# SuwoongHeo/neurecon

Hardware: AMD Instinct MI355X
Metric: rays/sec (4096 rays x 128 samples, 8-layer x256 SDF MLP) (higher is better)
Workload: dtype f16x3

## Files before the change

### neurecon_amd/csrc/nr_mlp.hip

```cpp
#include <algorithm>
#include <atomic>
#include <type_traits>
#include "nr_common.h"
#include "nr_mlp.h"
#include "nr_tgemm.h"

namespace nr {

using lds_ptr = __attribute__((address_space(3))) void*;

__device__ __forceinline__ void glds16(const char* gsrc, uint32_t lds_addr) {
  unsigned keep;
  asm volatile(
      "s_mov_b32 %0, m0\n\t"
      "s_mov_b32 m0, %2\n\t"
      "s_nop 0\n\t"
      "global_load_lds_dwordx4 %1, off\n\t"
      "s_mov_b32 m0, %0"
      : "=&s"(keep)
      : "v"(gsrc), "s"(lds_addr)
      : "memory");
}

__device__ __forceinline__ void glds16s(const char* sbase, uint32_t voff, uint32_t lds_addr) {
// ... 725 lines not shown
template <bool DERIV>
__device__ __forceinline__ void softplus3(float z, float& y, float& s) {
  const float t = z * 100.0f;
  const bool lin = t > 20.0f;
  const float ex = __builtin_amdgcn_exp2f(t * 1.44269504088896341f);
  const float u = 1.0f + ex;
  const float yy = __builtin_amdgcn_logf(u) * (0.693147180559945309f * 0.01f);
  y = lin ? z : yy;
  if constexpr (DERIV) s = lin ? 1.0f : ex * __builtin_amdgcn_rcpf(u);
}
__device__ __forceinline__ void softplus1(float z, float& y, float& s) {
  const float t = z * 144.269504088896341f;
  const float ex = __builtin_amdgcn_exp2f(t);
  const float u = ex + 1.0f;
  const bool lin = t > 28.8539008f;
  y = lin ? z : __builtin_amdgcn_logf(u) * (0.693147180559945309f * 0.01f);
  s = lin ? 1.0f : ex * __builtin_amdgcn_rcpf(u);
}
template <bool DERIV>
__device__ __forceinline__ void softplus_pk(float z0, float z1, float& y0, float& y1, float& s0, float& s1) {
  float d0, d1;
  softplus1(z0, y0, d0);
  softplus1(z1, y1, d1);
  if constexpr (DERIV) {
    s0 = d0;
    s1 = d1;
  }
}
__device__ __forceinline__ float4 fma4s(f32x4 a, float m, float4 b) {
  return make_float4(__builtin_fmaf(a[0], m, b.x), __builtin_fmaf(a[1], m, b.y), __builtin_fmaf(a[2], m, b.z),
                     __builtin_fmaf(a[3], m, b.w));
}

using gf4 = __attribute__((address_space(1))) f32x4;

constexpr int kNC = 1;
constexpr int kW4 = 8 / kNC;
constexpr int kT4 = 64 * kW4;
constexpr int kWPE = kW4 / 4;
constexpr int kSlabW = 2 * kNC * 1024;
constexpr int kSlab4 = kW4 * kSlabW;
constexpr int kLoad = 8;
static_assert(kLoad >= 1 && kLoad <= kW4, "loader waves");

typedef uint32_t u32x3 __attribute__((ext_vector_type(3)));
struct Pend4 {
  float4* base;
  uint32_t o[4];
  float4 v[4];
  int n;
  bool nt;
  bool b96;
  __device__ __forceinline__ int flush() {
    int issued = 0;
    if (base) {
      issued = n;
#pragma unroll
      for (int i = 0; i < 4; ++i) {
        if (i < n) {
          if (b96) {
            const uint32_t off = o[i];
            const u32x3 d = {__float_as_uint(v[i].x), __float_as_uint(v[i].y), __float_as_uint(v[i].z)};
            if (nt) asm volatile("global_store_dwordx3 %0, %1, %2 nt\n\ts_nop 1" : : "v"(off), "v"(d), "s"(base) : "memory");
            else asm volatile("global_store_dwordx3 %0, %1, %2\n\ts_nop 1" : : "v"(off), "v"(d), "s"(base) : "memory");
          } else {
            const uint32_t off = o[i] * 16u;
            const f32x4 d = tof(v[i]);
            if (nt) asm volatile("global_store_dwordx4 %0, %1, %2 nt\n\ts_nop 1" : : "v"(off), "v"(d), "s"(base) : "memory");
            else asm volatile("global_store_dwordx4 %0, %1, %2\n\ts_nop 1" : : "v"(off), "v"(d), "s"(base) : "memory");
          }
        }
      }
      base = nullptr;
    }
    return issued;
  }
  __device__ __forceinline__ void put(float4* b, int cnt, bool nontemporal, bool bytes96 = false) {
    base = b;
    n = cnt;
    nt = nontemporal;
    b96 = bytes96;
  }
};

constexpr int kSlabRing = 3;
constexpr int kFwdRing = 4;
constexpr int kTabBytes = 8 * 512;
constexpr bool kSlabNT = true;
constexpr bool kFeatNT = false;

template <int CBMAX, int RING = 3, int NW = kW4>
struct WStream4 {
  static_assert(RING == 3 || RING == 4, "weight ring depth");
  static constexpr int kRingN = RING;
  static constexpr int kLd = NW == kW4 ? kLoad : NW;
  char* lds;
  char* slab;
  int cur;
  int es;
  int er;
  int prev;
  char* tab;
  int tcur;
  __device__ __forceinline__ static int wave_id() { return __builtin_amdgcn_readfirstlane(threadIdx.x >> 6); }
  __device__ __forceinline__ static int next3(int i) { return i == 2 ? 0 : i + 1; }
  __device__ __forceinline__ static int nextr(int i) { return i == RING - 1 ? 0 : i + 1; }
  __device__ __forceinline__ int ahead_slot() const { return cur == 0 ? RING - 1 : cur - 1; }
  template <int BYTES>
  __device__ __forceinline__ static constexpr int pieces() { return (BYTES / 1024 + kLd - 1) / kLd; }
  __device__ __forceinline__ static int loader() { return wave_id() - (NW - kLd); }
  template <int BYTES>
  __device__ __forceinline__ static int npieces() { return loader() >= 0 ? pieces<BYTES>() : 0; }
  template <int BYTES>
  __device__ __forceinline__ void dma(const char* gsrc, int slot) {
    constexpr int NB = BYTES / 1024, NPW = pieces<BYTES>();
    const int wave = loader();
    if (wave < 0) return;
    const uint32_t voff = (threadIdx.x & 63) * 16;
    const int first = __builtin_amdgcn_readfirstlane(min(wave * NPW, NB - NPW));
    const char* g = uniform_ptr(gsrc) + first * 1024;
    const uint32_t base =
        __builtin_amdgcn_readfirstlane(lds_u32(lds) + (uint32_t)(slot * CBMAX) + (uint32_t)(first * 1024));
#pragma unroll
    for (int j = 0; j < NPW; j += 4) {
      const char* gj = g + j * 1024;
      const uint32_t mj = base + j * 1024;
      if (NPW - j >= 4)
        asm volatile(
            "s_mov_b32 m0, %2\n\ts_nop 0\n\t"
            "global_load_lds_dwordx4 %0, %1\n\t"
            "global_load_lds_dwordx4 %0, %1 offset:1024\n\t"
            "global_load_lds_dwordx4 %0, %1 offset:2048\n\t"
            "global_load_lds_dwordx4 %0, %1 offset:3072"
            :
            : "v"(voff), "s"(gj), "s"(mj)
            : "memory", "m0");
      else if (NPW - j == 3)
        asm volatile(
            "s_mov_b32 m0, %2\n\ts_nop 0\n\t"
            "global_load_lds_dwordx4 %0, %1\n\t"
            "global_load_lds_dwordx4 %0, %1 offset:1024\n\t"
            "global_load_lds_dwordx4 %0, %1 offset:2048"
            :
            : "v"(voff), "s"(gj), "s"(mj)
            : "memory", "m0");
      else if (NPW - j == 2)
        asm volatile(
            "s_mov_b32 m0, %2\n\ts_nop 0\n\t"
            "global_load_lds_dwordx4 %0, %1\n\t"
            "global_load_lds_dwordx4 %0, %1 offset:1024"
            :
            : "v"(voff), "s"(gj), "s"(mj)
            : "memory", "m0");
      else
        glds16m(gj, voff, mj);
    }
  }
  template <int B0, int B1>
  __device__ __forceinline__ void start(const char* g0, const char* g1) {
    static_assert(RING == 3, "start: the first RING - 1 chunks");
    cur = 0;
    es = 0;
    er = 0;
    prev = 0;
    dma<B0>(g0, 0);
    dma<B1>(g1, 1);
// ... 69 lines not shown
    return (const float4*)(lds + off);
  }
  __device__ __forceinline__ void flip(int n) {
    if constexpr (RING == 4) {
      wait_vmcnt(n + prev);
      prev = n;
    } else {
      wait_vmcnt(n);
    }
    __syncthreads();
    cur = nextr(cur);
  }
  __device__ __forceinline__ void flip_nowait() {
    __syncthreads();
    cur = nextr(cur);
  }
};

__device__ __forceinline__ f16x8 rd_frag(const float4* __restrict__ A, int i, int lane) {
  return as_h8(A[i * 64 + lane]);
}
template <int NS, class Stage>
__device__ __forceinline__ void mma4(const float4* __restrict__ A, const f16x8 (&bh)[kNC][12],
                                     const f16x8 (&bl)[kNC][12], f32x4 (&acc)[kNC][2], int lane, Stage&& stage) {
  f16x8 nh0 = rd_frag(A, 0, lane), nl0 = rd_frag(A, 1, lane);
  f16x8 nh1 = rd_frag(A, NS * 2, lane), nl1 = rd_frag(A, NS * 2 + 1, lane);
#pragma unroll
  for (int s = 0; s < NS; ++s) {
    const f16x8 h0 = nh0, l0 = nl0, h1 = nh1, l1 = nl1;
    if (s + 1 < NS) {
      nh0 = rd_frag(A, (s + 1) * 2, lane);
      nl0 = rd_frag(A, (s + 1) * 2 + 1, lane);
      nh1 = rd_frag(A, (NS + s + 1) * 2, lane);
      nl1 = rd_frag(A, (NS + s + 1) * 2 + 1, lane);
    }
    stage(s);
#pragma unroll
    for (int q = 0; q < kNC; ++q) {
      acc[q][0] = mfma16h(l0, bh[q][s], acc[q][0]);
      acc[q][1] = mfma16h(l1, bh[q][s], acc[q][1]);
      acc[q][0] = mfma16h(h0, bl[q][s], acc[q][0]);
      acc[q][1] = mfma16h(h1, bl[q][s], acc[q][1]);
      acc[q][0] = mfma16h(h0, bh[q][s], acc[q][0]);
      acc[q][1] = mfma16h(h1, bh[q][s], acc[q][1]);
    }
    if (s + 1 < NS) __builtin_amdgcn_sched_group_barrier(0x100, 4, 0);
    __builtin_amdgcn_sched_group_barrier(0x008, 6 * kNC, 0);
    __builtin_amdgcn_sched_barrier(0);
  }
}

struct Z4 {
  float4 z[kNC][2];
  float4 aux[2];
};

constexpr float kT = 144.26944f;
constexpr float kC = 0.0069314749f;

#ifdef NR_EXP_STAMPS
constexpr int kStampPh = 9;
constexpr int kStampSlot = 2048 * 8 * kStampPh;
__device__ unsigned long long g_nr_stamps[6 * kStampSlot];
__device__ __forceinline__ unsigned long long* stamp_lds() {
  __shared__ unsigned long long s_stamp[kW4 * kStampPh];
  return s_stamp;
}
__device__ __forceinline__ uint64_t stamp_now() { return __builtin_amdgcn_s_memtime(); }
__device__ __forceinline__ void stamp_add(int ph, uint64_t dt) {
  if ((threadIdx.x & 63) == 0) stamp_lds()[(threadIdx.x >> 6) * kStampPh + ph] += dt;
}
#define NR_STAMP(var) const uint64_t var = stamp_now()
#define NR_STAMP_VAR(var) uint64_t var = 0
#define NR_STAMP_SET(var) var = stamp_now()
#define NR_STAMP_ADD(ph, dt) stamp_add(ph, dt)
#else
#define NR_STAMP(var)
#define NR_STAMP_VAR(var)
#define NR_STAMP_SET(var)
#define NR_STAMP_ADD(ph, dt)
#endif

enum { kSlot = 0, kLean = 1, kTab = 2 };
template <int KB, int NBO, int NXT_CB, bool AUX, bool TS, int MODE = kSlot, int NXT_MODE = kSlot, class WS,
          class Pre, class Epi>
__device__ __forceinline__ void op4(WS& ws, const char* __restrict__ op, const char* nxt, const f16x8 (&bh)[kNC][12],
                                    const f16x8 (&bl)[kNC][12], const float (&xinv)[kNC], Pend4& pd, Pre&& pre,
                                    Epi&& epi, int lane, float winv = 0.0f) {
  constexpr int CB = chunk_bytes(KB);
  constexpr bool LEAN = MODE == kLean;
  constexpr int FB = MODE != kSlot ? weight_bytes(KB) : CB;
  constexpr int NXT_FB = NXT_MODE != kSlot ? NXT_CB - 1024 : NXT_CB;
  static_assert(!LEAN || (!AUX && !TS), "lean ops carry no per-row data");
  constexpr int NCH = NBO / 2;
  static_assert(MODE != kTab || NCH * 512 <= kTabBytes, "bias table entries");
  constexpr int LA = WS::kRingN - 1;
  static_assert(NCH >= 2, "the 2-ahead stream needs >= 2 chunks per op");
  const int g = lane >> 4;
  Z4 zq{};
#pragma unroll
  for (int c = 0; c < NCH; ++c) {
    const char* opc = op;
    const char* nxc = nxt;
    asm volatile("" : "+s"(opc), "+s"(nxc));
    NR_STAMP(t0);
    int npend = 0;
    if (c + LA < NCH) {
      ws.template issue<FB>(opc + (c + LA) * CB);
      npend = WS::template npieces<FB>();
    } else if (nxc) {
      ws.template issue<NXT_FB>(nxc + (c + LA - NCH) * NXT_CB);
      npend = WS::template npieces<NXT_FB>();
      if constexpr (NXT_MODE == kTab) {
        if (c + LA == NCH) {
          ws.template dma_tab<NXT_CB>(nxc, ws.tcur ^ 1);
          npend += WS::ntab();
        }
      }
    }
    npend += pre(c);
    npend += pd.flush();
    NR_STAMP(t1);
    const float4* A = ws.buf();
    f32x4 acc[kNC][2] = {};
    mma4<KB / 2>(A, bh, bl, acc, lane, [&](int st) {
      if (c > 0) {
#pragma unroll
        for (int e = 0; e < 8; ++e)
          if (e * (KB / 2) / 8 == st) epi(c - 1, zq, e);
      }
    });
    NR_STAMP(t2);
    float wi;
    float4 b0, b1;
    if constexpr (LEAN) {
      wi = winv;
      b0 = b1 = make_float4(0.f, 0.f, 0.f, 0.f);
    } else {
      const float4* S = MODE == kTab ? ws.tab_entry(c) : A + 2 * KB * 64;
      wi = S[8].x;
      if constexpr (TS) wi *= kT;
      b0 = S[(TS ? 24 : 0) + g];
      b1 = S[(TS ? 28 : 4) + g];
    }
#pragma unroll
    for (int q = 0; q < kNC; ++q) {
      const float inv = xinv[q] * wi;
      zq.z[q][0] = fma4s(acc[q][0], inv, b0);
      zq.z[q][1] = fma4s(acc[q][1], inv, b1);
    }
    if constexpr (AUX) {
      const float4* S = MODE == kTab ? ws.tab_entry(c) : A + 2 * KB * 64;
      zq.aux[0] = S[16 + g];
      zq.aux[1] = S[20 + g];
    }
#ifdef NR_EXP_STAMPS
    wait_vmcnt(npend);
    NR_STAMP(t3);
    ws.flip(npend);
    NR_STAMP(t4);
    stamp_add(0, t1 - t0);
    stamp_add(1, t2 - t1);
    stamp_add(2, t3 - t2);
    stamp_add(3, t4 - t3);
    stamp_add(4, 1);
#else
    ws.flip(npend);
#endif
  }
  pd.flush();
  if constexpr (MODE == kTab) ws.tcur ^= 1;
#pragma unroll
  for (int e = 0; e < 8; ++e) epi(NCH - 1, zq, e);
}

template <bool NABLA>
__device__ __forceinline__ void sp_pair(const Z4& zz, int q, int k, float4 (&y)[2], float4& s0, float4& s1) {
  const int o = k >> 1;
  const float4 z = zz.z[q][o];
  float4& s = o ? s1 : s0;
  if ((k & 1) == 0) softplus_pk<NABLA>(z.x, z.y, y[o].x, y[o].y, s.x, s.y);
  else softplus_pk<NABLA>(z.z, z.w, y[o].z, y[o].w, s.z, s.w);
}
__device__ __forceinline__ float4 mul4(float4 a, float4 b) { return make_float4(a.x * b.x, a.y * b.y, a.z * b.z, a.w * b.w); }
__device__ __forceinline__ uint32_t opaque_lane(int lane) {
  uint32_t l = (uint32_t)lane;
  asm volatile("" : "+v"(l));
  return l;
}
__device__ __forceinline__ void pend_chunk(Pend4& pd, float4* base, int first_blk, int lane, bool nt) {
  const uint32_t l = opaque_lane(lane);
#pragma unroll
  for (int i = 0; i < 2 * kNC; ++i) pd.o[i] = (kNC * first_blk + i) * 64 + l;
  pd.put(base, 2 * kNC, nt);
}
__device__ __forceinline__ void pend_chunk24(Pend4& pd, float4* layer, int c, int lane, bool nt) {
  const uint32_t l = opaque_lane(lane);
#pragma unroll
  for (int i = 0; i < 2 * kNC; ++i) pd.o[i] = (uint32_t)(c * kNC * kSlab24Chunk) + ((uint32_t)i * 64 + l) * 12u;
  pd.put(layer, 2 * kNC, nt, true);
}
__device__ __forceinline__ uint32_t code24(float c) { return (uint32_t)__builtin_fmaf(c, 8388608.0f, 0.5f); }
__device__ __forceinline__ float4 pack24(float c0, float c1, float c2, float c3) {
  const uint32_t u0 = code24(c0), u1 = code24(c1), u2 = code24(c2), u3 = code24(c3);
  return make_float4(__uint_as_float(u0 | (u1 << 24)), __uint_as_float((u1 >> 8) | (u2 << 16)),
                     __uint_as_float((u2 >> 16) | (u3 << 8)), 0.0f);
}
__device__ __forceinline__ float4 unpack24_mul(uint32_t w0, uint32_t w1, uint32_t w2, float4 g) {
  const float u0 = (float)(w0 & 0xFFFFFFu);
  const float u1 = (float)(__builtin_amdgcn_alignbit(w1, w0, 24) & 0xFFFFFFu);
  const float u2 = (float)(__builtin_amdgcn_alignbit(w2, w1, 16) & 0xFFFFFFu);
  const float u3 = (float)(w2 >> 8);
  constexpr float k = 1.0f / 8388608.0f;
  return make_float4(__builtin_fmaf(-(g.x * k), u0, g.x), __builtin_fmaf(-(g.y * k), u1, g.y),
                     __builtin_fmaf(-(g.z * k), u2, g.z), __builtin_fmaf(-(g.w * k), u3, g.w));
}


template <bool NABLA>
struct FwdEpi4 {
  static constexpr int NV = 8 * kNC;
  f16x8 (&oh)[kNC][12];
  f16x8 (&ol)[kNC][12];
  const float (&sc)[kNC];
  float4* sl;
  float (&mrun)[kNC];
  Pend4& pd;
  int lane;
  float e[NV], L[NV], m[NV];
  __device__ __forceinline__ static float zval(const Z4& zz, int i) {
    const float4 v = zz.z[i >> 3][(i >> 2) & 1];
    const int r = i & 3;
    return r == 0 ? v.x : (r == 1 ? v.y : (r == 2 ? v.z : v.w));
  }
  __device__ __forceinline__ void operator()(int c, const Z4& zz, int st) {
    if (st == 0) {
#pragma unroll
      for (int i = 0; i < NV; ++i) e[i] = fminf(zval(zz, i), 126.0f);
    } else if (st == 1) {
#pragma unroll
      for (int i = 0; i < NV; ++i) e[i] = __builtin_amdgcn_exp2f(e[i]);
    } else if (st == 2) {
#pragma unroll
      for (int i = 0; i < NV; ++i) e[i] = e[i] + 1.0f;
#pragma unroll
      for (int i = 0; i < NV / 2; ++i) L[i] = __builtin_amdgcn_logf(e[i]);
    } else if (st == 3) {
#pragma unroll
      for (int i = NV / 2; i < NV; ++i) L[i] = __builtin_amdgcn_logf(e[i]);
      if constexpr (NABLA) {
#pragma unroll
        for (int i = 0; i < NV / 2; ++i) e[i] = __builtin_amdgcn_rcpf(e[i]);
      }
    } else if (st == 4) {
#pragma unroll
      for (int i = 0; i < NV; ++i) m[i] = fmaxf(L[i], zval(zz, i));
      if constexpr (NABLA) {
#pragma unroll
        for (int i = NV / 2; i < NV; ++i) e[i] = __builtin_amdgcn_rcpf(e[i]);
      }
    } else if (st == 5) {
#pragma unroll
      for (int q = 0; q < kNC; ++q) {
        const int i = 8 * q;
        float r = mrun[q];
        r = __builtin_fmaxf(r, __builtin_fmaxf(m[i + 0], m[i + 1]));
        r = __builtin_fmaxf(r, __builtin_fmaxf(m[i + 2], m[i + 3]));
        r = __builtin_fmaxf(r, __builtin_fmaxf(m[i + 4], m[i + 5]));
        r = __builtin_fmaxf(r, __builtin_fmaxf(m[i + 6], m[i + 7]));
        mrun[q] = r;
      }
      if constexpr (NABLA) {
#pragma unroll
        for (int q = 0; q < kNC; ++q)
#pragma unroll
          for (int o = 0; o < 2; ++o) {
            const int i = (2 * q + o) * 4;
            pd.v[kNC * o + q] = pack24(e[i], e[i + 1], e[i + 2], e[i + 3]);
          }
      }
    } else if (st == 6) {
      split8a(make_float4(m[0], m[1], m[2], m[3]), make_float4(m[4], m[5], m[6], m[7]), sc[0] * kC, oh[0][c],
              ol[0][c]);
    } else {
      if constexpr (NABLA) pend_chunk24(pd, sl, c, lane, kSlabNT);
    }
  }
};

template <bool NABLA, bool FEAT>
struct F7Epi4 {
  f16x8 (&oh)[kNC][12];
  f16x8 (&ol)[kNC][12];
  const float (&sc)[kNC];
  float4* g7;
  float (&mrun)[kNC];
  float (&sdf_part)[kNC];
  Pend4& pd;
  int lane;
  float4 y[kNC][2], s[kNC][2];
  __device__ __forceinline__ void operator()(int c, const Z4& zz, int st) {
    const int q = st >> 2, k = st & 3;
    if (q < kNC) sp_pair<NABLA>(zz, q, k, y[q], s[q][0], s[q][1]);
    if (q < kNC && k == 3) {
      const float4 w0 = zz.aux[0], w1 = zz.aux[1];
      float sp = sdf_part[q];
      sp = fmaf(y[q][0].x, w0.x, sp); sp = fmaf(y[q][0].y, w0.y, sp);
      sp = fmaf(y[q][0].z, w0.z, sp); sp = fmaf(y[q][0].w, w0.w, sp);
      sp = fmaf(y[q][1].x, w1.x, sp); sp = fmaf(y[q][1].y, w1.y, sp);
      sp = fmaf(y[q][1].z, w1.z, sp); sp = fmaf(y[q][1].w, w1.w, sp);
      sdf_part[q] = sp;
      if constexpr (NABLA) {
        pd.v[q] = mul4(w0, s[q][0]);
        pd.v[kNC + q] = mul4(w1, s[q][1]);
      }
      if constexpr (FEAT) {
        mrun[q] = amax8(mrun[q], y[q][0], y[q][1]);
        split8a(y[q][0], y[q][1], sc[q], oh[q][c], ol[q][c]);
      }
    }
    if constexpr (NABLA)
      if (st == 7) pend_chunk(pd, g7, 2 * c, lane, kFeatNT);
  }
};

template <int NMAIN, class WS>
struct BwdEpi4 {
  f16x8 (&oh)[kNC][12];
  f16x8 (&ol)[kNC][12];
  const float (&sc)[kNC];
  WS& ws;
  float4* park;
  int park_blk;
  float (&mrun)[kNC];
  Pend4& pd;
  int lane;
  int plane;
  float4 y[kNC][2];
  __device__ __forceinline__ void operator()(int c, const Z4& zz, int st) {
    if (2 * c < NMAIN) {
      const int q = st >> 2, k = st & 3;
      if (q >= kNC) return;
      if (k < 2) {
        const uint4 sw = *(const uint4*)((const char*)ws.slab_read() + ((kNC * k + q) * 64 + lane) * 16);
        y[q][k] = unpack24_mul(sw.x, sw.y, sw.z, zz.z[q][k]);
      } else if (k == 2) {
        mrun[q] = amax8(mrun[q], y[q][0], y[q][1]);
      } else {
        split8a(y[q][0], y[q][1], sc[q], oh[q][c], ol[q][c]);
        if (q == kNC - 1) ws.slab_consumed();
      }
    } else if (st == 7) {
#pragma unroll
      for (int q = 0; q < kNC; ++q) {
        pd.v[q] = zz.z[q][0];
        pd.v[kNC + q] = zz.z[q][1];
      }
      pend_chunk(pd, park, park_blk + 2 * c - NMAIN, plane, false);
    }
  }
};

struct NoPre4 {
  __device__ __forceinline__ int operator()(int) const { return 0; }
};

template <bool NABLA, bool FEAT, int STAGE_>
constexpr bool kSdfClaim = NABLA && (STAGE_ == 2 || STAGE_ == 4 || (FEAT && STAGE_ == 0));

template <bool NABLA, bool FEAT, int STAGE_>
__global__ __attribute__((amdgpu_flat_work_group_size(STAGE_ == 3 ? 256 : kT4, STAGE_ == 3 ? 256 : kT4),
                          amdgpu_waves_per_eu(kWPE, kWPE)))
void sdf4_kernel(std::conditional_t<kSdfClaim<NABLA, FEAT, STAGE_>, SdfKArgsC, SdfKArgs> a) {
  constexpr int STAGE = STAGE_ == 3 ? 0 : (STAGE_ == 4 ? 2 : STAGE_);
  constexpr bool COMPACT = STAGE_ == 4;
  constexpr bool CLAIM = kSdfClaim<NABLA, FEAT, STAGE_>;
  constexpr int NW = STAGE_ == 3 ? 4 : kW4;
  static_assert(STAGE_ != 3 || (!NABLA && !FEAT), "narrow tiles: forward-only launches");
  static_assert(STAGE == 0 || (NABLA && !FEAT), "deferred nablas: no feature");
  constexpr int PPW = 16 * kNC * NW;
#ifdef NR_EXP_ROW_ENC
  constexpr bool ENC4 = false;
#else
  constexpr bool ENC4 = NABLA && STAGE != 1 && !(!FEAT && STAGE_ == 0);
#endif
  constexpr int CB = chunk_bytes(18);
  constexpr int C16 = chunk_bytes(16), C4 = chunk_bytes(4), C14 = chunk_bytes(14), C18 = chunk_bytes(18);
  static_assert((size_t)kW4 * kNC * kSlabColBytes <= kScratchPerWG, "per-workgroup slab scratch");
  constexpr bool SLABS = NABLA && STAGE != 1;
  constexpr int RING = SLABS ? 3 : kFwdRing;
  constexpr bool TABF = !SLABS;
  constexpr int FM = TABF ? kTab : kSlot;
  constexpr int LDSB = RING * CB + (SLABS ? kSlabRing * kSlab4 : 0) + (TABF ? 2 * kTabBytes : 0);
  __shared__ __attribute__((aligned(16))) char smem[LDSB + (CLAIM ? 16 : 0)];
  static_assert(LDSB + (CLAIM ? 16 : 0) <= 160 * 1024, "LDS budget");
  static_assert(!TABF || RING * CB + 2 * kTabBytes == LDSB, "the bias table follows the weight ring");
  WStream4<CB, RING, NW> ws{smem, SLABS ? smem + RING * CB : nullptr, 0, 0, 0, 0, TABF ? smem + RING * CB : nullptr, 0};
  const int lane = threadIdx.x & 63, wave = __builtin_amdgcn_readfirstlane(threadIdx.x >> 6);
  const int j = lane & 15, g = lane >> 4;
  const char* W = a.packed;
  auto OP = [&](int i) {
    const char* w = W;
    asm volatile("" : "+s"(w));
    return w + sdf_op_off(i);
  };
  auto OPF8 = [&]() {
    const char* w = a.f8_alt;
    asm volatile("" : "+s"(w));
    return w ? w : OP(F8);
  };
  const float b8 = *(const float*)(W + a.L.misc_off);
  float4* escr = uniform_ptr((float4*)((char*)a.scratch + (size_t)(blockIdx.x * kW4 + wave) * (kNC * kSlabColBytes)));
  auto slab = [&](int l) {
    char* e = (char*)escr;
    asm volatile("" : "+s"(e));
    return (float4*)(e + l * kNC * kSlab24Layer);
  };

#ifdef NR_EXP_STAMPS
  if ((threadIdx.x & 63) == 0)
    for (int i = 0; i < kStampPh; ++i) stamp_lds()[wave * kStampPh + i] = 0;
#endif
  constexpr bool LEANR = STAGE == 2 || (NABLA && FEAT);
  constexpr int W16 = weight_bytes(16);
  if constexpr (STAGE == 2) ws.template start<W16, W16>(OP(B7), OP(B7) + C16);
  else if constexpr (TABF)
    ws.template start<weight_bytes(4), weight_bytes(4), weight_bytes(4), C4>(OP(F0), OP(F0) + C4, OP(F0) + 2 * C4, OP(F0));
  else ws.template start<C4, C4>(OP(F0), OP(F0) + C4);
  Pend4 pd{};
  NoPre4 nopre;
  const float kSpSlack = 0.0070f;

  const int64_t Pn = COMPACT      ? ((int64_t)(*a.n_tiles) + 15) / 16 * 16
                     : STAGE == 2 ? (int64_t)(*a.n_tiles) * kPointsPerWG / kW4
                                  : (a.P_dev ? min(a.P, (int64_t)(*a.P_dev) * a.P_mult) : a.P);
  int* claim = nullptr;
  if constexpr (CLAIM) claim = a.claim;
  int* const claim_lds = (int*)(smem + LDSB);
  int64_t next = 0;
  for (int64_t base = (int64_t)blockIdx.x * PPW; base < Pn; base = claim ? next : base + (int64_t)gridDim.x * PPW) {
    bool has_next = base + (int64_t)gridDim.x * PPW < Pn;
    int claimed = 0;
    if (claim && threadIdx.x == 0) claimed = atomicAdd(claim, 1);
    NR_STAMP_VAR(ts0);
    NR_STAMP_VAR(ts1);
    NR_STAMP_VAR(te0);
    NR_STAMP_SET(ts0);
    int64_t p0 = base + wave * 16 * kNC;
    int plane = lane;
    uint32_t soff = 0;
    int64_t pl = 0;
    bool listed = true;
    if constexpr (COMPACT) {
      const int64_t n = *a.n_tiles;
      const int64_t w0 = p0 < n ? p0 : n - 16;
      const int e = a.tiles[w0 + j];
      const int e0 = __builtin_amdgcn_readfirstlane(a.tiles[w0]);
      listed = p0 < n && e >= 0;
      pl = e >= 0 ? e : e0;
      const uint32_t rt = (uint32_t)((pl >> 4) - (e0 >> 4)), js = (uint32_t)(pl & 15);
      plane = (int)(rt * (uint32_t)(kSlabColBytes / 16) + js + 16u * (uint32_t)g);
      soff = rt * (uint32_t)kSlabColBytes + (js + 16u * (uint32_t)g) * (uint32_t)kSlabVB;
      escr = uniform_ptr((float4*)((char*)a.slabs + (size_t)(e0 >> 4) * kSlabColBytes));
    } else if constexpr (STAGE == 2) {
      const int64_t ti = min(p0 / 16, (int64_t)(*a.n_tiles) - 1);
      const int64_t tile = a.tiles[ti];
      escr = uniform_ptr((float4*)((char*)a.slabs + (size_t)tile * kSlabColBytes));
      p0 = p0 / 16 < (int64_t)(*a.n_tiles) ? tile * 16 : a.P;
    } else if constexpr (STAGE == 1) {
      escr = uniform_ptr((float4*)((char*)a.slabs + (size_t)(p0 / 16) * kSlabColBytes));
    }
    const int64_t Pv = STAGE == 2 ? a.P : Pn;
    int64_t pq[kNC];
    bool valid[kNC];
    float xs[kNC][3];
#pragma unroll
    for (int q = 0; q < kNC; ++q) {
      const int64_t p = p0 + 16 * q + j;
      if constexpr (COMPACT) {
        valid[q] = listed;
        pq[q] = pl;
      } else {
        valid[q] = p < Pv;
        pq[q] = valid[q] ? p : Pv - 1;
      }
      xs[q][0] = a.pts[pq[q] * 3 + 0];
      xs[q][1] = a.pts[pq[q] * 3 + 1];
      xs[q][2] = a.pts[pq[q] * 3 + 2];
    }
    if (claim && threadIdx.x == 0) *claim_lds = claimed;
    float4 E[kNC][4];
    float mE[kNC], xinv[kNC];
    f16x8 Uh[kNC][12], Ul[kNC][12], Vh[kNC][12], Vl[kNC][12];
    float mrun[kNC], m_in[kNC];
    auto next_scales = [&](int kb, float extra, const float (&floor_max)[kNC], float (&sc)[kNC]) {
      const float4 v = TABF ? ws.tab_entry(0)[8] : ws.buf()[2 * kb * 64 + 8];
#pragma unroll
      for (int q = 0; q < kNC; ++q) sc[q] = bound_scale(fmaxf(fmaf(v.y, m_in[q], v.z) + extra, floor_max[q]));
    };
    struct OpScal {
      float winv, R, B;
    };
    auto op_scal = [&](int opi) {
      const char* w = W;
      asm volatile("" : "+s"(w));
      typedef __attribute__((address_space(4))) const float cfloat;
      cfloat* rb = (cfloat*)(w + a.L.bound_off + 8 * opi);
      return OpScal{*(cfloat*)(w + a.L.winv_off + 4 * opi), rb[0], rb[1]};
    };
    auto finish = [&](const float (&sc)[kNC], float mscale = 1.0f) {
#pragma unroll
      for (int q = 0; q < kNC; ++q) {
        m_in[q] = max4_groups(mrun[q]) * mscale;
        mrun[q] = 0.0f;
        xinv[q] = 1.0f / sc[q];
      }
    };
    float zero2[kNC];
#pragma unroll
    for (int q = 0; q < kNC; ++q) zero2[q] = 0.0f;
    if constexpr (STAGE != 2) {
#pragma unroll
    for (int q = 0; q < kNC; ++q) {
      if constexpr (ENC4) {
        const int ge = (int)opaque_lane(g), je = (int)opaque_lane(j);
        Enc4 t;
        enc_eval(t, xs[q], ge);
        E[q][0] = enc_rows<0>(t, xs[q], ge, je);
        E[q][1] = enc_rows<1>(t, xs[q], ge, je);
        E[q][2] = enc_rows<2>(t, xs[q], ge, je);
        E[q][3] = enc_rows<3>(t, xs[q], ge, je);
      } else {
#pragma unroll
        for (int b = 0; b < 4; ++b) {
          const int f = 16 * b + 4 * g;
          E[q][b] = make_float4(embed_feature(f + 0, xs[q][0], xs[q][1], xs[q][2], a.nfreq),
                                embed_feature(f + 1, xs[q][0], xs[q][1], xs[q][2], a.nfreq),
                                embed_feature(f + 2, xs[q][0], xs[q][1], xs[q][2], a.nfreq),
                                embed_feature(f + 3, xs[q][0], xs[q][1], xs[q][2], a.nfreq));
        }
      }
      mE[q] = max4_groups(amax8(amax8(0.0f, E[q][0], E[q][1]), E[q][2], E[q][3]));
      const float sE = bound_scale(mE[q]);
      split8a(E[q][0], E[q][1], sE, Uh[q][0], Ul[q][0]);
      split8a(E[q][2], E[q][3], sE, Uh[q][1], Ul[q][1]);
      xinv[q] = 1.0f / sE;
    }
    float4* epark = slab(7);
    if constexpr (NABLA) {
      const uint32_t l = opaque_lane(lane);
#pragma unroll
      for (int q = 0; q < kNC; ++q)
#pragma unroll
        for (int b = 0; b < 4; ++b) {
          const uint32_t off = (((12 + b) * kNC + q) * 64 + l) * 16u;
          const f32x4 d = tof(E[q][b]);
          asm volatile("global_store_dwordx4 %0, %1, %2\n\ts_nop 1" : : "v"(off), "v"(d), "s"(epark) : "memory");
        }
    }
#pragma unroll
    for (int q = 0; q < kNC; ++q) {
      mrun[q] = 0.0f;
      m_in[q] = mE[q];
    }
    auto fwd_epi = [&](f16x8(&oh)[kNC][12], f16x8(&ol)[kNC][12], const float (&sc)[kNC], float4* sl) {
      return FwdEpi4<NABLA>{oh, ol, sc, sl, mrun, pd, lane};
    };

    NR_STAMP_SET(ts1);
    {
      float sc[kNC];
      next_scales(4, kSpSlack, zero2, sc);
      op4<4, 16, C16, false, true, FM, FM>(ws, OP(F0), OP(F1), Uh, Ul, xinv, pd, nopre, fwd_epi(Vh, Vl, sc, slab(0)), lane);
      finish(sc, kC);
    }
    {
      float sc[kNC];
      next_scales(16, kSpSlack, zero2, sc);
      op4<16, 16, C16, false, true, FM, FM>(ws, OP(F1), OP(F2), Vh, Vl, xinv, pd, nopre, fwd_epi(Uh, Ul, sc, slab(1)), lane);
      finish(sc, kC);
    }
    {
      float sc[kNC];
      next_scales(16, kSpSlack, zero2, sc);
      op4<16, 16, C16, false, true, FM, FM>(ws, OP(F2), OP(F3), Uh, Ul, xinv, pd, nopre, fwd_epi(Vh, Vl, sc, slab(2)), lane);
      finish(sc, kC);
    }
    {
      float sc[kNC];
      next_scales(16, kSpSlack, mE, sc);
      op4<16, 14, C18, false, true, FM, FM>(ws, OP(F3), OP(F4), Vh, Vl, xinv, pd, nopre, fwd_epi(Uh, Ul, sc, slab(3)), lane);
      if constexpr (NABLA) {
        asm volatile("s_waitcnt vmcnt(0)" ::: "memory");
#pragma unroll
        for (int q = 0; q < kNC; ++q)
#pragma unroll
          for (int b = 0; b < 4; ++b) E[q][b] = fromf(*((const gf4*)epark + ((12 + b) * kNC + q) * 64 + lane));
      }
#pragma unroll
      for (int q = 0; q < kNC; ++q) {
        split8a(E[q][0], E[q][1], sc[q], Uh[q][7], Ul[q][7]);
        split8a(E[q][2], E[q][3], sc[q], Uh[q][8], Ul[q][8]);
        mrun[q] = fmaxf(mrun[q], mE[q] * (1.0f / kC));
      }
      finish(sc, kC);
    }
    {
      float sc[kNC];
      next_scales(18, kSpSlack, zero2, sc);
      op4<18, 16, C16, false, true, FM, FM>(ws, OP(F4), OP(F5), Uh, Ul, xinv, pd, nopre, fwd_epi(Vh, Vl, sc, slab(4)), lane);
      finish(sc, kC);
    }
    {
      float sc[kNC];
      next_scales(16, kSpSlack, zero2, sc);
      op4<16, 16, C16, false, true, FM, FM>(ws, OP(F5), OP(F6), Vh, Vl, xinv, pd, nopre, fwd_epi(Uh, Ul, sc, slab(5)), lane);
      finish(sc, kC);
    }
    {
      float sc[kNC];
      next_scales(16, kSpSlack, zero2, sc);
      op4<16, 16, C16, false, true, FM, FM>(ws, OP(F6), OP(F7), Uh, Ul, xinv, pd, nopre, fwd_epi(Vh, Vl, sc, slab(6)), lane);
      finish(sc, kC);
    }
    float sdf_part[kNC];
#pragma unroll
    for (int q = 0; q < kNC; ++q) sdf_part[q] = 0.0f;
    {
      float sc[kNC];
      next_scales(16, kSpSlack, zero2, sc);
      F7Epi4<NABLA, FEAT> epi{Uh, Ul, sc, slab(7), mrun, sdf_part, pd, lane};
      constexpr int NXT = ((NABLA && STAGE == 0) || FEAT) ? C16 : C4;
      const char* n;
      if constexpr (FEAT) n = OPF8();
      else n = (NABLA && STAGE == 0) ? OP(B7) : (has_next ? OP(F0) : nullptr);
      op4<16, 16, NXT, true, false, FM, FM>(ws, OP(F7), n, Vh, Vl, xinv, pd, nopre, epi, lane);
      finish(sc);
    }
    NR_STAMP_SET(te0);
#pragma unroll
    for (int q = 0; q < kNC; ++q) {
      const float sdf = wave_sum4(sdf_part[q]) + b8;
      if (valid[q] && g == 0) a.sdf[p0 + 16 * q + j] = sdf;
    }
    if constexpr (FEAT) {
      const int64_t pf = p0 < Pn ? p0 : Pn - 1;
      float4* fb = uniform_ptr((float4*)(a.feature + pf * 256));
      uint32_t frow[kNC];
#pragma unroll
      for (int q = 0; q < kNC; ++q) frow[q] = (uint32_t)(pq[q] - pf);
      auto epi = [&](int c, const Z4& zz, int st) {
        if (st != 7) return;
#pragma unroll
        for (int q = 0; q < kNC; ++q) {
          pd.v[2 * q] = zz.z[q][0];
          pd.v[2 * q + 1] = zz.z[q][1];
          const uint32_t r = opaque_lane(frow[q] * 64 + g);
          pd.o[2 * q] = r + (2 * c) * 4;
          pd.o[2 * q + 1] = r + (2 * c + 1) * 4;
        }
        pd.put(fb, 2 * kNC, kFeatNT);
      };
      constexpr int NXT = NABLA ? C16 : C4;
      const char* n = NABLA ? OP(B7) : (has_next ? OP(F0) : nullptr);
      op4<16, 16, NXT, false, false, FM, NABLA ? (LEANR ? kLean : kSlot) : FM>(ws, OPF8(), n, Uh, Ul, xinv, pd, nopre, epi,
                                                                               lane);
      NR_STAMP_SET(te0);
    }
    }
    if constexpr (NABLA && STAGE == 1) {
      pd.flush();
    }
    if constexpr (NABLA && STAGE != 1) {
      pd.flush();
      asm volatile("s_waitcnt vmcnt(0)" ::: "memory");
      OpScal osn{};
      if constexpr (LEANR) osn = op_scal(B7);
      float4* g7 = slab(7);
#pragma unroll
      for (int q = 0; q < kNC; ++q) {
        float4 G[16];
#pragma unroll
        for (int b = 0; b < 16; ++b) G[b] = fromf(*((const gf4*)g7 + (kNC * b + q) * 64 + (COMPACT ? plane : lane)));
        float m = 0.0f;
#pragma unroll
        for (int b = 0; b < 16; b += 2) m = amax8(m, G[b], G[b + 1]);
        m_in[q] = max4_groups(m);
        mrun[q] = 0.0f;
        const float sc = bound_scale(m_in[q]);
#pragma unroll
        for (int s = 0; s < 8; ++s) split8a(G[2 * s], G[2 * s + 1], sc, Uh[q][s], Ul[q][s]);
        xinv[q] = 1.0f / sc;
      }
      float4* park = slab(7);
      if constexpr (COMPACT) ws.stage_slab(slab(6), 0, soff);
      else ws.stage_slab(slab(6), 0);
      auto bwd = [&](auto kb_tag, auto nbo_tag, auto nmain_tag, auto nxt_tag, auto nxl_tag, int opi, const char* nxt,
                     f16x8(&ih)[kNC][12], f16x8(&il)[kNC][12], f16x8(&oh)[kNC][12], f16x8(&ol)[kNC][12], int lcur,
                     int park_blk, int lnext) {
        constexpr int KBo = decltype(kb_tag)::value, NBOo = decltype(nbo_tag)::value;
        constexpr int NMAIN = decltype(nmain_tag)::value, NXC = decltype(nxt_tag)::value;
        constexpr bool NXL = decltype(nxl_tag)::value;
        const OpScal os = osn;
        float sc[kNC];
        if constexpr (LEANR) {
          if (opi != B0) osn = op_scal(opi + 1);
#pragma unroll
          for (int q = 0; q < kNC; ++q) sc[q] = bound_scale(fmaxf(fmaf(os.R, m_in[q], os.B) + 0.0f, zero2[q]));
        } else {
          next_scales(KBo, 0.0f, zero2, sc);
        }
        auto pre = [&](int c) -> int {
          if constexpr (COMPACT) {
            if (2 * (c + 1) < NMAIN) return ws.stage_slab(slab(lcur), c + 1, soff);
            if (c + 1 == NBOo / 2 && lnext >= 0) return ws.stage_slab(slab(lnext), 0, soff);
          } else {
            if (2 * (c + 1) < NMAIN) return ws.stage_slab(slab(lcur), c + 1);
            if (c + 1 == NBOo / 2 && lnext >= 0) return ws.stage_slab(slab(lnext), 0);
          }
          return 0;
        };
        BwdEpi4<NMAIN, decltype(ws)> epi{oh, ol, sc, ws, park, park_blk, mrun, pd, lane, COMPACT ? plane : lane};
        constexpr int RM = LEANR ? kLean : kSlot, RMN = (LEANR && NXL) ? kLean : kSlot;
        op4<KBo, NBOo, NXC, false, false, RM, RMN>(ws, OP(opi), nxt, ih, il, xinv, pd, pre, epi, lane, os.winv);
        finish(sc);
      };
      using I0 = std::integral_constant<int, 0>;
      using I4 = std::integral_constant<int, 4>;
      using I14 = std::integral_constant<int, 14>;
      using I16 = std::integral_constant<int, 16>;
      using I18 = std::integral_constant<int, 18>;
      using IC16 = std::integral_constant<int, C16>;
      using IC14 = std::integral_constant<int, C14>;
      using IC4 = std::integral_constant<int, C4>;
      using LeanNext = std::true_type;
      using SlotNext = std::false_type;
      if constexpr (STAGE == 2) {
        NR_STAMP_SET(ts1);
      }
      bwd(I16{}, I16{}, I16{}, IC16{}, LeanNext{}, B7, OP(B6), Uh, Ul, Vh, Vl, 6, 0, 5);
      bwd(I16{}, I16{}, I16{}, IC16{}, LeanNext{}, B6, OP(B5), Vh, Vl, Uh, Ul, 5, 0, 4);
      bwd(I16{}, I16{}, I16{}, IC16{}, LeanNext{}, B5, OP(B4), Uh, Ul, Vh, Vl, 4, 0, 3);
      bwd(I16{}, I18{}, I14{}, IC14{}, LeanNext{}, B4, OP(B3), Vh, Vl, Uh, Ul, 3, 0, 2);
      bwd(I14{}, I16{}, I16{}, IC16{}, LeanNext{}, B3, OP(B2), Uh, Ul, Vh, Vl, 2, 0, 1);
      bwd(I16{}, I16{}, I16{}, IC16{}, LeanNext{}, B2, OP(B1), Vh, Vl, Uh, Ul, 1, 0, 0);
      bwd(I16{}, I16{}, I16{}, IC16{}, LeanNext{}, B1, OP(B0), Uh, Ul, Vh, Vl, 0, 0, -1);
      if (claim) {
        next = (int64_t)(gridDim.x + __builtin_amdgcn_readfirstlane(*claim_lds)) * PPW;
        has_next = next < Pn;
      }
      if constexpr (STAGE == 2) bwd(I16{}, I4{}, I0{}, IC16{}, LeanNext{}, B0, has_next ? OP(B7) : nullptr, Vh, Vl, Uh, Ul, 0, 4, -1);
      else bwd(I16{}, I4{}, I0{}, IC4{}, SlotNext{}, B0, has_next ? OP(F0) : nullptr, Vh, Vl, Uh, Ul, 0, 4, -1);
      NR_STAMP_SET(te0);
      pd.flush();
      asm volatile("s_waitcnt vmcnt(0)" ::: "memory");
#pragma unroll
      for (int q = 0; q < kNC; ++q) {
        float n0 = 0.f, n1 = 0.f, n2 = 0.f;
        auto grad = [&](int b) {
          const float4 u = fromf(*((const gf4*)park + (kNC * b + q) * 64 + (COMPACT ? plane : lane)));
          const float4 v = fromf(*((const gf4*)park + (kNC * (4 + b) + q) * 64 + (COMPACT ? plane : lane)));
          return make_float4(fadd(v.x, u.x), fadd(v.y, u.y), fadd(v.z, u.z), fadd(v.w, u.w));
        };
        if constexpr (ENC4) {
          const int ge = (int)opaque_lane(g), je = (int)opaque_lane(j);
          Enc4 t;
          enc_eval(t, xs[q], ge);
          const float4 g0 = grad(0), g1 = grad(1), g2 = grad(2);
          enc_row_bwd<0>(t, g0.x, ge, je, n0, n1, n2);
          enc_row_bwd<1>(t, g0.y, ge, je, n0, n1, n2);
          enc_row_bwd<2>(t, g0.z, ge, je, n0, n1, n2);
          enc_row_bwd<3>(t, g0.w, ge, je, n0, n1, n2);
          enc_row_bwd<16>(t, g1.x, ge, je, n0, n1, n2);
          enc_row_bwd<17>(t, g1.y, ge, je, n0, n1, n2);
          enc_row_bwd<18>(t, g1.z, ge, je, n0, n1, n2);
          enc_row_bwd<19>(t, g1.w, ge, je, n0, n1, n2);
          enc_row_bwd<32>(t, g2.x, ge, je, n0, n1, n2);
          enc_row_bwd<33>(t, g2.y, ge, je, n0, n1, n2);
          enc_row_bwd<34>(t, g2.z, ge, je, n0, n1, n2);
          enc_row_bwd<35>(t, g2.w, ge, je, n0, n1, n2);
        } else {
#pragma unroll
          for (int b = 0; b < 4; ++b) {
            const float4 gr = grad(b);
            const int f = 16 * b + 4 * g;
            embed_backward(f + 0, gr.x, xs[q][0], xs[q][1], xs[q][2], a.nfreq, n0, n1, n2);
            embed_backward(f + 1, gr.y, xs[q][0], xs[q][1], xs[q][2], a.nfreq, n0, n1, n2);
            embed_backward(f + 2, gr.z, xs[q][0], xs[q][1], xs[q][2], a.nfreq, n0, n1, n2);
            embed_backward(f + 3, gr.w, xs[q][0], xs[q][1], xs[q][2], a.nfreq, n0, n1, n2);
          }
        }
        n0 = wave_sum4(n0);
        n1 = wave_sum4(n1);
        n2 = wave_sum4(n2);
        if (valid[q] && g == 0) {
          const int64_t p = COMPACT ? pq[q] : p0 + 16 * q + j;
          a.nabla[p * 3 + 0] = n0;
          a.nabla[p * 3 + 1] = n1;
          a.nabla[p * 3 + 2] = n2;
        }
      }
    }
    NR_STAMP(te1);
    NR_STAMP_ADD(6, ts1 - ts0);
    NR_STAMP_ADD(7, te1 - te0);
    NR_STAMP_ADD(8, te1 - ts0);
  }
  pd.flush();
  wait_vmcnt(0);
#ifdef NR_EXP_STAMPS
  if ((threadIdx.x & 63) == 0 && blockIdx.x < 2048)
    for (int i = 0; i < kStampPh; ++i) {
      const unsigned long long v = stamp_lds()[wave * kStampPh + i];
      g_nr_stamps[(blockIdx.x * kW4 + wave) * kStampPh + i] = v;
      g_nr_stamps[(1 + STAGE_) * kStampSlot + (blockIdx.x * kW4 + wave) * kStampPh + i] = v;
    }
#endif
}


template <int P, bool NABLA>
__global__ __launch_bounds__(kThreads) void siren_sdf_kernel(SdfKArgs a) {
  constexpr int CB = chunk_bytes(16);
  __shared__ __attribute__((aligned(16))) char smem[kRing * CB + (NABLA ? 2 * kSlabChunk : 0)];
  WStream<CB> ws{smem, NABLA ? smem + kRing * CB : nullptr, 0, 0, 0};
  const int lane = threadIdx.x & 63, wave = __builtin_amdgcn_readfirstlane(threadIdx.x >> 6);
  const int j = lane & 15, g = lane >> 4;
  const SdfLayout& L = a.L;
  const char* W = a.packed;
  auto OP = [&](int i) { return W + L.op_off[i]; };
  auto OPB = [&](int i) { return (int)L.op_bytes[i]; };
  const float* wl = (const float*)(W + L.w8row0_off);
  const float bl = *(const float*)(W + L.misc_off);
  float4* escr = uniform_ptr(a.scratch + (size_t)(blockIdx.x * kWaves + wave) * (8 * 16 * 64));
  const bool want_feat = a.feature != nullptr;
// ... 1908 lines not shown
```

Measured before the change: 732,200.

## Overlap slab-7 gradient reload with F8 and prefetch F3 embeddings

In the fused forward+backward SDF MLP kernel, layer-7 gradient blocks are now loaded chunk by chunk during the F8 op and split into f16 hi/lo operands inside its epilogue. Their max-abs scale is tracked in the F7 epilogue, so the backward pass can start without a serial reload of the slab, a max-reduction and a split. Embedding blocks for F3 are also issued from inside the op loop, and only the needed vmcnt is waited on instead of draining to zero. op4 gains a top hook and returns the count of outstanding loads. The aim is to hide global-load latency at the forward/backward turn, at the cost of more live registers and more complex buffer swapping, which may hurt occupancy.

```diff
diff --git a/neurecon_amd/csrc/nr_mlp.hip b/neurecon_amd/csrc/nr_mlp.hip
--- a/neurecon_amd/csrc/nr_mlp.hip
+++ b/neurecon_amd/csrc/nr_mlp.hip
@@ -831,6 +831,19 @@
     b96 = bytes96;
   }
 };
+
+__device__ __forceinline__ void ld_blocks2(const char* base, uint32_t voff, float4& b0, float4& b1) {
+  f32x4 v0, v1;
+  asm volatile("global_load_dwordx4 %0, %1, %2" : "=v"(v0) : "v"(voff), "s"(base) : "memory");
+  asm volatile("global_load_dwordx4 %0, %1, %2 offset:1024" : "=v"(v1) : "v"(voff), "s"(base) : "memory");
+  b0 = fromf(v0);
+  b1 = fromf(v1);
+}
+__device__ __forceinline__ void pin4(float4& v) {
+  f32x4 t = tof(v);
+  asm volatile("" : "+v"(t));
+  v = fromf(t);
+}
 
 constexpr int kSlabRing = 3;
 constexpr int kFwdRing = 4;
@@ -1066,11 +1079,14 @@
 #endif
 
 enum { kSlot = 0, kLean = 1, kTab = 2 };
+struct NoPre4 {
+  __device__ __forceinline__ int operator()(int) const { return 0; }
+};
 template <int KB, int NBO, int NXT_CB, bool AUX, bool TS, int MODE = kSlot, int NXT_MODE = kSlot, class WS,
-          class Pre, class Epi>
-__device__ __forceinline__ void op4(WS& ws, const char* __restrict__ op, const char* nxt, const f16x8 (&bh)[kNC][12],
-                                    const f16x8 (&bl)[kNC][12], const float (&xinv)[kNC], Pend4& pd, Pre&& pre,
-                                    Epi&& epi, int lane, float winv = 0.0f) {
+          class Pre, class Epi, class Top = NoPre4>
+__device__ __forceinline__ int op4(WS& ws, const char* __restrict__ op, const char* nxt, const f16x8 (&bh)[kNC][12],
+                                   const f16x8 (&bl)[kNC][12], const float (&xinv)[kNC], Pend4& pd, Pre&& pre,
+                                   Epi&& epi, int lane, float winv = 0.0f, Top&& top = Top{}) {
   constexpr int CB = chunk_bytes(KB);
   constexpr bool LEAN = MODE == kLean;
   constexpr int FB = MODE != kSlot ? weight_bytes(KB) : CB;
@@ -1082,19 +1098,21 @@
   static_assert(NCH >= 2, "the 2-ahead stream needs >= 2 chunks per op");
   const int g = lane >> 4;
   Z4 zq{};
+  int behind = 0;
 #pragma unroll
   for (int c = 0; c < NCH; ++c) {
     const char* opc = op;
     const char* nxc = nxt;
     asm volatile("" : "+s"(opc), "+s"(nxc));
     NR_STAMP(t0);
-    int npend = 0;
+    const int ntop = top(c);
+    int npend = ntop;
     if (c + LA < NCH) {
       ws.template issue<FB>(opc + (c + LA) * CB);
-      npend = WS::template npieces<FB>();
+      npend += WS::template npieces<FB>();
     } else if (nxc) {
       ws.template issue<NXT_FB>(nxc + (c + LA - NCH) * NXT_CB);
-      npend = WS::template npieces<NXT_FB>();
+      npend += WS::template npieces<NXT_FB>();
       if constexpr (NXT_MODE == kTab) {
         if (c + LA == NCH) {
           ws.template dma_tab<NXT_CB>(nxc, ws.tcur ^ 1);
@@ -1104,6 +1122,7 @@
     }
     npend += pre(c);
     npend += pd.flush();
+    if (c == NCH - 1) behind = npend - ntop;
     NR_STAMP(t1);
     const float4* A = ws.buf();
     f32x4 acc[kNC][2] = {};
@@ -1152,10 +1171,11 @@
     ws.flip(npend);
 #endif
   }
-  pd.flush();
+  behind += pd.flush();
   if constexpr (MODE == kTab) ws.tcur ^= 1;
 #pragma unroll
   for (int e = 0; e < 8; ++e) epi(NCH - 1, zq, e);
+  return behind;
 }
 
 template <bool NABLA>
@@ -1280,6 +1300,7 @@
   float4* g7;
   float (&mrun)[kNC];
   float (&sdf_part)[kNC];
+  float (&gmax)[kNC];
   Pend4& pd;
   int lane;
   float4 y[kNC][2], s[kNC][2];
@@ -1297,6 +1318,10 @@
       if constexpr (NABLA) {
         pd.v[q] = mul4(w0, s[q][0]);
         pd.v[kNC + q] = mul4(w1, s[q][1]);
+        if constexpr (FEAT) {
+          gmax[q] = amax8(gmax[q], pd.v[q], pd.v[kNC + q]);
+          asm volatile("" : "+v"(gmax[q]), "+v"(sdf_part[q]));
+        }
       }
       if constexpr (FEAT) {
         mrun[q] = amax8(mrun[q], y[q][0], y[q][1]);
@@ -1345,10 +1370,6 @@
   }
 };
 
-struct NoPre4 {
-  __device__ __forceinline__ int operator()(int) const { return 0; }
-};
-
 template <bool NABLA, bool FEAT, int STAGE_>
 constexpr bool kSdfClaim = NABLA && (STAGE_ == 2 || STAGE_ == 4 || (FEAT && STAGE_ == 0));
 
@@ -1368,6 +1389,8 @@
 #else
   constexpr bool ENC4 = NABLA && STAGE != 1 && !(!FEAT && STAGE_ == 0);
 #endif
+  constexpr bool TURN8 = NABLA && FEAT && STAGE_ == 0;
+  constexpr bool RELOAD3 = NABLA && ((FEAT && STAGE_ == 0) || STAGE_ == 1);
   constexpr int CB = chunk_bytes(18);
   constexpr int C16 = chunk_bytes(16), C4 = chunk_bytes(4), C14 = chunk_bytes(14), C18 = chunk_bytes(18);
   static_assert((size_t)kW4 * kNC * kSlabColBytes <= kScratchPerWG, "per-workgroup slab scratch");
@@ -1503,6 +1526,12 @@
     float zero2[kNC];
 #pragma unroll
     for (int q = 0; q < kNC; ++q) zero2[q] = 0.0f;
+    float gm[kNC], gsc[kNC];
+#pragma unroll
+    for (int q = 0; q < kNC; ++q) {
+      gm[q] = 0.0f;
+      gsc[q] = 1.0f;
+    }
     if constexpr (STAGE != 2) {
 #pragma unroll
     for (int q = 0; q < kNC; ++q) {
@@ -1573,13 +1602,41 @@
     {
       float sc[kNC];
       next_scales(16, kSpSlack, mE, sc);
-      op4<16, 14, C18, false, true, FM, FM>(ws, OP(F3), OP(F4), Vh, Vl, xinv, pd, nopre, fwd_epi(Uh, Ul, sc, slab(3)), lane);
+      int behind = 0;
+      auto top3 = [&](int c) -> int {
+        if (c != 6) return 0;
+        const char* gb = (const char*)epark + 12 * 1024;
+        const uint32_t voff = opaque_lane(lane) * 16u;
+        ld_blocks2(gb, voff, E[0][0], E[0][1]);
+        ld_blocks2(gb + 2048, voff, E[0][2], E[0][3]);
+        return 4;
+      };
+      static_assert(!RELOAD3 || kNC == 1, "F3's embedding loads: one column per wave");
+      if constexpr (RELOAD3)
+        behind = op4<16, 14, C18, false, true, FM, FM>(ws, OP(F3), OP(F4), Vh, Vl, xinv, pd, nopre,
+                                                       fwd_epi(Uh, Ul, sc, slab(3)), lane, 0.0f, top3);
+      else op4<16, 14, C18, false, true, FM, FM>(ws, OP(F3), OP(F4), Vh, Vl, xinv, pd, nopre, fwd_epi(Uh, Ul, sc, slab(3)), lane);
       if constexpr (NABLA) {
-        asm volatile("s_waitcnt vmcnt(0)" ::: "memory");
+        NR_STAMP(tr0);
+        if constexpr (RELOAD3) {
+          wait_vmcnt(behind);
+#pragma unroll
+          for (int b = 0; b < 4; ++b) pin4(E[0][b]);
+        } else {
+          asm volatile("s_waitcnt vmcnt(0)" ::: "memory");
+#pragma unroll
+          for (int q = 0; q < kNC; ++q)
+#pragma unroll
+            for (int b = 0; b < 4; ++b) E[q][b] = fromf(*((const gf4*)epark + ((12 + b) * kNC + q) * 64 + lane));
+        }
+#ifdef NR_EXP_STAMPS
 #pragma unroll
         for (int q = 0; q < kNC; ++q)
 #pragma unroll
-          for (int b = 0; b < 4; ++b) E[q][b] = fromf(*((const gf4*)epark + ((12 + b) * kNC + q) * 64 + lane));
+          for (int b = 0; b < 4; ++b) pin4(E[q][b]);
+        NR_STAMP(tr1);
+        NR_STAMP_ADD(5, tr1 - tr0);
+#endif
       }
 #pragma unroll
       for (int q = 0; q < kNC; ++q) {
@@ -1613,13 +1670,20 @@
     {
       float sc[kNC];
       next_scales(16, kSpSlack, zero2, sc);
-      F7Epi4<NABLA, FEAT> epi{Uh, Ul, sc, slab(7), mrun, sdf_part, pd, lane};
+      F7Epi4<NABLA, FEAT> epi{Uh, Ul, sc, slab(7), mrun, sdf_part, gm, pd, lane};
       constexpr int NXT = ((NABLA && STAGE == 0) || FEAT) ? C16 : C4;
       const char* n;
       if constexpr (FEAT) n = OPF8();
       else n = (NABLA && STAGE == 0) ? OP(B7) : (has_next ? OP(F0) : nullptr);
       op4<16, 16, NXT, true, false, FM, FM>(ws, OP(F7), n, Vh, Vl, xinv, pd, nopre, epi, lane);
       finish(sc);
+      if constexpr (TURN8) {
+#pragma unroll
+        for (int q = 0; q < kNC; ++q) {
+          gm[q] = max4_groups(gm[q]);
+          gsc[q] = bound_scale(gm[q]);
+        }
+      }
     }
     NR_STAMP_SET(te0);
 #pragma unroll
@@ -1633,7 +1697,28 @@
       uint32_t frow[kNC];
 #pragma unroll
       for (int q = 0; q < kNC; ++q) frow[q] = (uint32_t)(pq[q] - pf);
+      float4 G8[8][2];
+      auto pre8 = [&](int c) -> int {
+        if (c > 6) return 0;
+        const char* gb = (const char*)slab(7) + c * 2048;
+        const uint32_t voff = opaque_lane(lane) * 16u;
+        ld_blocks2(gb, voff, G8[c][0], G8[c][1]);
+        if (c < 6) return 2;
+        ld_blocks2(gb + 2048, voff, G8[7][0], G8[7][1]);
+        return 4;
+      };
+      auto split_g7 = [&](int s) {
+        pin4(G8[s][0]);
+        pin4(G8[s][1]);
+#pragma unroll
+        for (int q = 0; q < kNC; ++q) split8a(G8[s][0], G8[s][1], gsc[q], Vh[q][s], Vl[q][s]);
+      };
+      static_assert(!TURN8 || kNC == 1, "F8's slab-7 loads: one column per wave");
       auto epi = [&](int c, const Z4& zz, int st) {
+        if constexpr (TURN8) {
+          if (st == 3 && c >= 1) split_g7(c - 1);
+          if (st == 5 && c == 7) split_g7(7);
+        }
         if (st != 7) return;
 #pragma unroll
         for (int q = 0; q < kNC; ++q) {
@@ -1647,8 +1732,9 @@
       };
       constexpr int NXT = NABLA ? C16 : C4;
       const char* n = NABLA ? OP(B7) : (has_next ? OP(F0) : nullptr);
-      op4<16, 16, NXT, false, false, FM, NABLA ? (LEANR ? kLean : kSlot) : FM>(ws, OPF8(), n, Uh, Ul, xinv, pd, nopre, epi,
-                                                                               lane);
+      constexpr int NM = NABLA ? (LEANR ? kLean : kSlot) : FM;
+      if constexpr (TURN8) op4<16, 16, NXT, false, false, FM, NM>(ws, OPF8(), n, Uh, Ul, xinv, pd, pre8, epi, lane);
+      else op4<16, 16, NXT, false, false, FM, NM>(ws, OPF8(), n, Uh, Ul, xinv, pd, nopre, epi, lane);
       NR_STAMP_SET(te0);
     }
     }
@@ -1661,20 +1747,29 @@
       OpScal osn{};
       if constexpr (LEANR) osn = op_scal(B7);
       float4* g7 = slab(7);
-#pragma unroll
-      for (int q = 0; q < kNC; ++q) {
-        float4 G[16];
-#pragma unroll
-        for (int b = 0; b < 16; ++b) G[b] = fromf(*((const gf4*)g7 + (kNC * b + q) * 64 + (COMPACT ? plane : lane)));
-        float m = 0.0f;
-#pragma unroll
-        for (int b = 0; b < 16; b += 2) m = amax8(m, G[b], G[b + 1]);
-        m_in[q] = max4_groups(m);
-        mrun[q] = 0.0f;
-        const float sc = bound_scale(m_in[q]);
-#pragma unroll
-        for (int s = 0; s < 8; ++s) split8a(G[2 * s], G[2 * s + 1], sc, Uh[q][s], Ul[q][s]);
-        xinv[q] = 1.0f / sc;
+      if constexpr (TURN8) {
+#pragma unroll
+        for (int q = 0; q < kNC; ++q) {
+          m_in[q] = gm[q];
+          mrun[q] = 0.0f;
+          xinv[q] = 1.0f / gsc[q];
+        }
+      } else {
+#pragma unroll
+        for (int q = 0; q < kNC; ++q) {
+          float4 G[16];
+#pragma unroll
+          for (int b = 0; b < 16; ++b) G[b] = fromf(*((const gf4*)g7 + (kNC * b + q) * 64 + (COMPACT ? plane : lane)));
+          float m = 0.0f;
+#pragma unroll
+          for (int b = 0; b < 16; b += 2) m = amax8(m, G[b], G[b + 1]);
+          m_in[q] = max4_groups(m);
+          mrun[q] = 0.0f;
+          const float sc = bound_scale(m_in[q]);
+#pragma unroll
+          for (int s = 0; s < 8; ++s) split8a(G[2 * s], G[2 * s + 1], sc, Uh[q][s], Ul[q][s]);
+          xinv[q] = 1.0f / sc;
+        }
       }
       float4* park = slab(7);
       if constexpr (COMPACT) ws.stage_slab(slab(6), 0, soff);
@@ -1722,19 +1817,21 @@
       if constexpr (STAGE == 2) {
         NR_STAMP_SET(ts1);
       }
-      bwd(I16{}, I16{}, I16{}, IC16{}, LeanNext{}, B7, OP(B6), Uh, Ul, Vh, Vl, 6, 0, 5);
-      bwd(I16{}, I16{}, I16{}, IC16{}, LeanNext{}, B6, OP(B5), Vh, Vl, Uh, Ul, 5, 0, 4);
-      bwd(I16{}, I16{}, I16{}, IC16{}, LeanNext{}, B5, OP(B4), Uh, Ul, Vh, Vl, 4, 0, 3);
-      bwd(I16{}, I18{}, I14{}, IC14{}, LeanNext{}, B4, OP(B3), Vh, Vl, Uh, Ul, 3, 0, 2);
-      bwd(I14{}, I16{}, I16{}, IC16{}, LeanNext{}, B3, OP(B2), Uh, Ul, Vh, Vl, 2, 0, 1);
-      bwd(I16{}, I16{}, I16{}, IC16{}, LeanNext{}, B2, OP(B1), Vh, Vl, Uh, Ul, 1, 0, 0);
-      bwd(I16{}, I16{}, I16{}, IC16{}, LeanNext{}, B1, OP(B0), Uh, Ul, Vh, Vl, 0, 0, -1);
+      f16x8(&Xh)[kNC][12] = TURN8 ? Vh : Uh, (&Xl)[kNC][12] = TURN8 ? Vl : Ul;
+      f16x8(&Yh)[kNC][12] = TURN8 ? Uh : Vh, (&Yl)[kNC][12] = TURN8 ? Ul : Vl;
+      bwd(I16{}, I16{}, I16{}, IC16{}, LeanNext{}, B7, OP(B6), Xh, Xl, Yh, Yl, 6, 0, 5);
+      bwd(I16{}, I16{}, I16{}, IC16{}, LeanNext{}, B6, OP(B5), Yh, Yl, Xh, Xl, 5, 0, 4);
+      bwd(I16{}, I16{}, I16{}, IC16{}, LeanNext{}, B5, OP(B4), Xh, Xl, Yh, Yl, 4, 0, 3);
+      bwd(I16{}, I18{}, I14{}, IC14{}, LeanNext{}, B4, OP(B3), Yh, Yl, Xh, Xl, 3, 0, 2);
+      bwd(I14{}, I16{}, I16{}, IC16{}, LeanNext{}, B3, OP(B2), Xh, Xl, Yh, Yl, 2, 0, 1);
+      bwd(I16{}, I16{}, I16{}, IC16{}, LeanNext{}, B2, OP(B1), Yh, Yl, Xh, Xl, 1, 0, 0);
+      bwd(I16{}, I16{}, I16{}, IC16{}, LeanNext{}, B1, OP(B0), Xh, Xl, Yh, Yl, 0, 0, -1);
       if (claim) {
         next = (int64_t)(gridDim.x + __builtin_amdgcn_readfirstlane(*claim_lds)) * PPW;
         has_next = next < Pn;
       }
-      if constexpr (STAGE == 2) bwd(I16{}, I4{}, I0{}, IC16{}, LeanNext{}, B0, has_next ? OP(B7) : nullptr, Vh, Vl, Uh, Ul, 0, 4, -1);
-      else bwd(I16{}, I4{}, I0{}, IC4{}, SlotNext{}, B0, has_next ? OP(F0) : nullptr, Vh, Vl, Uh, Ul, 0, 4, -1);
+      if constexpr (STAGE == 2) bwd(I16{}, I4{}, I0{}, IC16{}, LeanNext{}, B0, has_next ? OP(B7) : nullptr, Yh, Yl, Xh, Xl, 0, 4, -1);
+      else bwd(I16{}, I4{}, I0{}, IC4{}, SlotNext{}, B0, has_next ? OP(F0) : nullptr, Yh, Yl, Xh, Xl, 0, 4, -1);
       NR_STAMP_SET(te0);
       pd.flush();
       asm volatile("s_waitcnt vmcnt(0)" ::: "memory");
```

Result: no change. 735,900 (median of 6 runs) (+0.5%).
